# ipastore/glue-factory-colon

Measured on AMD Instinct MI355X. Metric: image-pairs/sec (SuperPoint+LightGlue, 1024 kpts, 640x480), higher is better.
Workload: dtype f32; 1 GPU; SuperPoint-open + LightGlue, 1024 kpts, 640x480 synthetic pairs (BASELINE.json configs[1]); keypoints=1024, parallelism=dp1 (pairs sharded, one final gather), weights=name-seeded seed 0 (no network), pairs_gathered=32, rccl_ranks=1

## Files before the change

glue-factory-colon_amd/csrc/conv_wino43.hip:

```cpp
#include "common.h"

#define S4_TW 32
#define S4_TH 16
#define S4_PR 18
#define S4_PC 34
#define S4_PITCH 36
#define S4_KC 16
#define S4_PLANE (S4_PR * S4_PITCH * 8)
#define S4_PATCH (2 * S4_PLANE)
#define S4_NPIX (S4_PR * S4_PC)
#define S4_IMR 20
#define S4_IMC 36
#define S4_EX (6 * 2 * 32 * 32)
#define S4_THREADS 768
#ifndef S4_DIAG
#define S4_DIAG 0
#endif
#if S4_DIAG & 1
static unsigned long long* g_s4_diag = nullptr;
extern "C" void gfc_diag_set_stem43_stamps(void* p) { g_s4_diag = (unsigned long long*)p; }
#define S4_T(v_) const unsigned long long v_ = __builtin_readcyclecounter()
#else
#define S4_T(v_) do {} while (0)
#endif

struct Stem43Args {
  const float* x;
  const float* w;
  const float* bias;
  const float* scale;
  const float* shift;
  float* y;
  int B, H, W;
  int tiles_x, tiles_y;
  const float* w1;
  const float* b1;
  const float* s1;
  const float* t1;
#if S4_DIAG & 1
  unsigned long long* diag;
#endif
};

__global__ void pack_conv3x3_wino43_kernel(const float* __restrict__ w, float* __restrict__ out, int cout, int cin) {
  const int idx = blockIdx.x * blockDim.x + threadIdx.x;
  if (idx >= cout * cin) return;
  const int ci = idx % cin, co = idx / cin;
  double g[3][3];
  for (int r = 0; r < 3; ++r)
    for (int c = 0; c < 3; ++c) g[r][c] = (double)w[((size_t)co * cin + ci) * 9 + r * 3 + c];
  const double G[6][3] = {{1.0 / 4, 0.0, 0.0},           {-1.0 / 6, -1.0 / 6, -1.0 / 6}, {-1.0 / 6, 1.0 / 6, -1.0 / 6},
                          {1.0 / 24, 1.0 / 12, 1.0 / 6}, {1.0 / 24, -1.0 / 12, 1.0 / 6}, {0.0, 0.0, 1.0}};
  double t[6][3];
  for (int i = 0; i < 6; ++i)
    for (int c = 0; c < 3; ++c) t[i][c] = G[i][0] * g[0][c] + G[i][1] * g[1][c] + G[i][2] * g[2][c];
  const int nt = co / 32, l31 = co % 32;
  const int kg = ci / 8, h = (ci % 8) / 4, s = ci % 4;
  const int lane = 32 * h + l31;
  const int nkg = cin / 8, ntn = cout / 32;
  for (int xi = 0; xi < 6; ++xi)
    for (int nu = 0; nu < 6; ++nu) {
      const double u = t[xi][0] * G[nu][0] + t[xi][1] * G[nu][1] + t[xi][2] * G[nu][2];
      const size_t o = ((((((size_t)xi * nkg + kg) * ntn + nt) * 2 + (s >> 1)) * 6 + nu) * 64 + lane) * 2 + (s & 1);
      out[o] = (float)u;
    }
}

extern "C" int gfc_pack_conv3x3_wino43(const float* w_oihw, float* w_packed, int cout, int cin, void* stream) {
  if (!w_oihw || !w_packed || cout != 64 || cin != 64) return GFC_ERR_INVALID;
  const int total = cout * cin;
  hipLaunchKernelGGL(pack_conv3x3_wino43_kernel, dim3((total + 255) / 256), dim3(256), 0, (hipStream_t)stream, w_oihw,
                     w_packed, cout, cin);
  GFC_LAUNCH_CHECK();
  return GFC_OK;
}

__device__ __forceinline__ float4 f4_scale(float s, float4 a) { return make_float4(s * a.x, s * a.y, s * a.z, s * a.w); }
__device__ __forceinline__ float4 f4_fma(float s, float4 a, float4 b) {
  return make_float4(fmaf(s, a.x, b.x), fmaf(s, a.y, b.y), fmaf(s, a.z, b.z), fmaf(s, a.w, b.w));
}
__device__ __forceinline__ float4 f4_addv(float4 a, float4 b) { return make_float4(a.x + b.x, a.y + b.y, a.z + b.z, a.w + b.w); }
__device__ __forceinline__ float4 f4_subv(float4 a, float4 b) { return make_float4(a.x - b.x, a.y - b.y, a.z - b.z, a.w - b.w); }
__device__ __forceinline__ float4 f4_max(float4 a, float4 b) {
  return make_float4(fmaxf(a.x, b.x), fmaxf(a.y, b.y), fmaxf(a.z, b.z), fmaxf(a.w, b.w));
}

typedef float v2f __attribute__((ext_vector_type(2)));
__device__ __forceinline__ v2f v2_fma(float s, v2f a, v2f b) { return v2f{fmaf(s, a.x, b.x), fmaf(s, a.y, b.y)}; }
__device__ __forceinline__ v2f v2_mul(float s, v2f a) { return v2f{s * a.x, s * a.y}; }
typedef const volatile __attribute__((address_space(3))) v2f* lds_v2f_ptr;
__device__ __forceinline__ v2f lds_pair(const float* p) { return *(lds_v2f_ptr)(p); }

__global__ __launch_bounds__(S4_THREADS, 1) void stem_wino43_kernel(Stem43Args args) {
  const float* const a_x = args.x;
  const float* const a_w = args.w;
  float* const a_y = args.y;
  const int a_B = args.B, a_H = args.H, a_W = args.W, a_tiles_x = args.tiles_x, a_tiles_y = args.tiles_y;
  extern __shared__ __attribute__((aligned(16))) float smem[];
  float* bufA = smem;
  float* bufB = smem + S4_PATCH;
  float* bufC = smem + 2 * S4_PATCH;
  float* img_s = smem + 2 * S4_PATCH + S4_EX;
  float* c1_s = img_s + S4_IMR * S4_IMC;
  float* c2_s = c1_s + 768;

  const int tid = threadIdx.x, lane = tid & 63;
  const int wave = __builtin_amdgcn_readfirstlane(tid >> 6);
  const int xi = wave % 6, nt = wave / 6;
  const int phase = wave >> 2;
  const int l31 = lane & 31, h = lane >> 5;
  const int ty = l31 >> 3, tx = l31 & 7;

  const int per_img = a_tiles_x * a_tiles_y;
  const int nitems = per_img * a_B;

  for (int i = tid; i < 768; i += S4_THREADS)
    c1_s[i] = i < 576 ? args.w1[i] : i < 640 ? args.b1[i - 576] : i < 704 ? (args.s1 ? args.s1[i - 640] : 1.f)
                                                                       : (args.t1 ? args.t1[i - 704] : 0.f);

  if (tid < 192)
    c2_s[tid] = tid < 64 ? args.bias[tid] : tid < 128 ? (args.scale ? args.scale[tid - 64] : 1.f) : (args.shift ? args.shift[tid - 128] : 0.f);

  auto load_img = [&](int it) __attribute__((always_inline)) -> float {
    int t_ = tid;
    asm volatile("" : "+v"(t_));
    const int im_r = (t_ * 1821) >> 16, im_c = t_ - im_r * S4_IMC;
    if (t_ >= S4_IMR * S4_IMC || it >= nitems) return 0.f;
    const int b = it / per_img, t = it - b * per_img;
    const int gy = (t / a_tiles_x) * S4_TH - 2 + im_r, gx = (t % a_tiles_x) * S4_TW - 2 + im_c;
    return (gy >= 0 && gy < a_H && gx >= 0 && gx < a_W) ? a_x[((size_t)b * a_H + gy) * a_W + gx] : 0.f;
  };

  const float2* wbase = reinterpret_cast<const float2*>(a_w) + (size_t)(xi * 32 + nt * 2) * 6 * 64;
  auto bfrag = [&](int hk, int nu) __attribute__((always_inline)) -> float2 {
    const float2* blk = wbase + (size_t)((hk >> 1) * 4 + (hk & 1)) * 6 * 64;
    return blk[nu * 64 + lane];
  };

  const bool three = xi == 0 || xi == 5;
  const int rP = three ? (xi == 0 ? 0 : 1) : (xi == 3 ? 3 : 1);
  const int rQ = three ? rP + 2 : (xi == 1 || xi == 2 ? 2 : (xi == 3 ? 1 : 3));
  const int rR = three ? rP + 4 : (xi == 1 ? 3 : 4);
  const int rS = xi == 1 ? 4 : (xi == 2 ? 3 : 2);
  const float c0 = three ? 4.f : (xi == 1 ? -4.f : xi == 2 ? 4.f : 2.f);
  const float c1 = three ? -5.f : (xi == 1 ? 1.f : -1.f);
  const float c2 = xi == 1 ? 1.f : -1.f;
  const int pix0 = (4 * ty * S4_PITCH + tx) * 8;
  const int offA = pix0 + 2 * ((2 * h) ^ ty), offB = pix0 + 2 * ((2 * h) ^ ((ty + 1) & 3));
  constexpr int COLOFF[6] = {0, 9 * 8, 18 * 8, 27 * 8, 1 * 8, 10 * 8};
  const int ro0 = rP * S4_PITCH * 8, ro1 = rQ * S4_PITCH * 8, ro2 = rR * S4_PITCH * 8, ro3 = rS * S4_PITCH * 8;
  const bool hiR = rR >= 4, hiS = rS >= 4;

#if S4_DIAG & 1
  unsigned long long dg[10] = {0, 0, 0, 0, 0, 0, 0, 0, 0, 0};
  const unsigned long long dg_t0 = __builtin_readcyclecounter();
#endif
  auto conv1a_unit = [&](int u, int ntile, int y0, int x0, float* dst_lo, float* dst_hi) __attribute__((always_inline)) {
    int ln = lane;
    asm volatile("" : "+v"(ln));
    S4_T(tc0);
    const int l31 = ln & 31, h = ln >> 5;
    const int ch = 32 * ntile + l31;
    const float* cb = c1_s + h * 64 + ch;
    const bool edge = u >= 18;
    const int idx_in = min(32 * (u - 18) + l31, 35);
    const float* ip = img_s + (edge ? (idx_in >> 1) * S4_IMC + 32 + (idx_in & 1) : u * S4_IMC + l31);
    f32x16 d;
#pragma unroll
    for (int r = 0; r < 16; ++r) d[r] = 0.f;
    constexpr int T0[5] = {0, 2, S4_IMC + 1, 2 * S4_IMC, 2 * S4_IMC + 2};
    constexpr int T1[5] = {1, S4_IMC, S4_IMC + 2, 2 * S4_IMC + 1, 2 * S4_IMC + 2};
#pragma unroll
    for (int s = 0; s < 5; ++s) {
      const float a0 = ip[T0[s]], a1 = s == 4 ? 1.f : ip[T1[s]];
      d = mfma32(h ? a1 : a0, cb[s * 128], d);
    }
    const float sc = c1_s[640 + ch], sh = c1_s[704 + ch];
#if S4_DIAG & 1
    float probe_ = fmaxf(d[0], 0.f);
    asm volatile("" : "+v"(probe_));
    S4_T(tc1);
    dg[8] += tc1 - tc0;
#endif
    float* dst = (l31 & 16) ? dst_hi : dst_lo;
    const int c16 = l31 & 15;
    const int cofs = (c16 >> 3) * S4_PLANE + (c16 & 1), cpr = (c16 >> 1) & 3;
    if (!edge) {
      const int gy = y0 - 1 + u;
      const bool row_in = gy >= 0 && gy < a_H;
      float* o = dst + cofs + (u * S4_PITCH + h) * 8 + 2 * (cpr ^ ((u >> 2) & 3));
      if (row_in && x0 >= 1 && x0 + 32 < a_W) {
#pragma unroll
        for (int r = 0; r < 16; ++r) {
          const int rr = (r & 3) + 8 * (r >> 2);
          o[((rr & 3) * 9 + (rr >> 2)) * 8] = fmaxf(d[r], 0.f) * sc + sh;
        }
      } else {
        const int gx0 = x0 - 1 + 4 * h;
#pragma unroll
        for (int r = 0; r < 16; ++r) {
          const int rr = (r & 3) + 8 * (r >> 2);
          const float v = (row_in && (unsigned)(gx0 + rr) < (unsigned)a_W) ? fmaxf(d[r], 0.f) * sc + sh : 0.f;
          o[((rr & 3) * 9 + (rr >> 2)) * 8] = v;
        }
      }
    } else {
      const int ib = 32 * (u - 18) + 4 * h;
#pragma unroll
      for (int r = 0; r < 16; ++r) {
        const int idx = ib + (r & 3) + 8 * (r >> 2);
        const bool real = idx < 36;
        const int p = real ? idx >> 1 : 17, cpos = real ? 8 + 9 * (idx & 1) : 35;
        const int gy = y0 - 1 + p, gx = x0 + 31 + (idx & 1);
        const float v = (gy >= 0 && gy < a_H && gx < a_W) ? fmaxf(d[r], 0.f) * sc + sh : 0.f;
        dst[cofs + (p * S4_PITCH + cpos) * 8 + 2 * (cpr ^ ((p >> 2) & 3))] = v;
      }
    }
  };
  auto conv1a_at_half = [&](int half, int ntile, int y0, int x0, float* dst_lo, float* dst_hi) __attribute__((always_inline)) {
    if (half == phase) conv1a_unit(wave, ntile, y0, x0, dst_lo, dst_hi);
    else if (half == phase + 1 && wave + 12 < 20) conv1a_unit(wave + 12, ntile, y0, x0, dst_lo, dst_hi);
  };
  int item = blockIdx.x;
  int y0, x0, b;
  {
    const float v0 = load_img(item);
    if (tid < S4_IMR * S4_IMC) img_s[tid] = v0;
    b = item / per_img;
    const int t_ = item - b * per_img;
    y0 = (t_ / a_tiles_x) * S4_TH; x0 = (t_ % a_tiles_x) * S4_TW;
    __syncthreads();
#pragma unroll 1
    for (int half = 0; half < 4; ++half) conv1a_at_half(half, 0, y0, x0, bufA, bufB);
  }
  float imv = load_img(item + gridDim.x);
  __syncthreads();

  for (; item < nitems; item += gridDim.x) {
    S4_T(t_top);
#if S4_DIAG & 1
    unsigned long long t_prev = t_top;
#endif
    const int nitem = item + gridDim.x;
    const bool have_next = nitem < nitems;
    const int nb_ = nitem / per_img, nt_ = nitem - nb_ * per_img;
    const int ny0 = (nt_ / a_tiles_x) * S4_TH, nx0 = (nt_ % a_tiles_x) * S4_TW;

    f32x16 acc[6];
#pragma unroll
    for (int nu = 0; nu < 6; ++nu)
#pragma unroll
      for (int r = 0; r < 16; ++r) acc[nu][r] = 0.f;

#pragma unroll 1
    for (int c = 0; c < 4; ++c) {
      const float* ps = (c & 1) == 0 ? (c == 0 ? bufA : bufA) : (c == 1 ? bufB : bufC);
      if (c == 2) {
        if (tid < S4_IMR * S4_IMC) img_s[tid] = imv;
        imv = load_img(nitem + gridDim.x);
      }
      S4_T(te);
#if S4_DIAG & 1
      unsigned long long cv_cycles = 0;
      dg[0] += te - t_prev;
#endif
#pragma unroll 1
      for (int half = 0; half < 4; ++half) {
        const int g = half >> 1, hh = half & 1;
        if ((c & 1) && (c == 1 || have_next)) {
          S4_T(tu);
          conv1a_at_half(half, c == 1 ? 1 : 0, c == 1 ? y0 : ny0, c == 1 ? x0 : nx0, bufA, c == 1 ? bufC : bufB);
#if S4_DIAG & 1
          cv_cycles += __builtin_readcyclecounter() - tu;
#endif
        }
        __builtin_amdgcn_sched_barrier(0);
        S4_T(tha);
        float2 bq[6];
#pragma unroll
        for (int nu = 0; nu < 6; ++nu) bq[nu] = bfrag(4 * c + half, nu);
        const float* pl = ps + g * S4_PLANE;
        const float* pA = pl + (offA ^ (2 * hh));
        const float* pB = pl + (offB ^ (2 * hh));
        const float* q0 = pA + ro0;
        const float* q1 = pA + ro1;
        const float* q2 = (hiR ? pB : pA) + ro2;
        const float* q3 = (hiS ? pB : pA) + ro3;
        v2f tr[6];
        if (three) {
          v2f d[2][3];
#pragma unroll
          for (int j = 0; j < 2; ++j) { d[j][0] = lds_pair(q0 + COLOFF[j]); d[j][1] = lds_pair(q1 + COLOFF[j]); d[j][2] = lds_pair(q2 + COLOFF[j]); }
#pragma unroll
          for (int j = 0; j < 6; ++j) {
            __builtin_amdgcn_sched_barrier(0);
            tr[j] = v2_fma(c1, d[j & 1][1], v2_mul(c0, d[j & 1][0])) + d[j & 1][2];
            if (j + 2 < 6) { d[j & 1][0] = lds_pair(q0 + COLOFF[j + 2]); d[j & 1][1] = lds_pair(q1 + COLOFF[j + 2]); d[j & 1][2] = lds_pair(q2 + COLOFF[j + 2]); }
          }
        } else {
          v2f d[2][4];
#pragma unroll
          for (int j = 0; j < 2; ++j) {
            d[j][0] = lds_pair(q0 + COLOFF[j]); d[j][1] = lds_pair(q1 + COLOFF[j]);
            d[j][2] = lds_pair(q2 + COLOFF[j]); d[j][3] = lds_pair(q3 + COLOFF[j]);
          }
#pragma unroll
          for (int j = 0; j < 6; ++j) {
            __builtin_amdgcn_sched_barrier(0);
            tr[j] = v2_fma(c0, v2_fma(c1, d[j & 1][1], d[j & 1][0]), v2_fma(c2, d[j & 1][3], d[j & 1][2]));
            if (j + 2 < 6) {
              d[j & 1][0] = lds_pair(q0 + COLOFF[j + 2]); d[j & 1][1] = lds_pair(q1 + COLOFF[j + 2]);
              d[j & 1][2] = lds_pair(q2 + COLOFF[j + 2]); d[j & 1][3] = lds_pair(q3 + COLOFF[j + 2]);
            }
          }
        }
        __builtin_amdgcn_sched_barrier(0);
        v2f v[6];
        {
          const v2f s12 = tr[1] + tr[2], d12 = tr[1] - tr[2], s34 = tr[3] + tr[4], d34 = tr[3] - tr[4];
          const v2f e31 = tr[3] - tr[1], e42 = tr[4] - tr[2];
          v[0] = v2_fma(-5.f, tr[2], v2_fma(4.f, tr[0], tr[4]));
          v[1] = v2_fma(-4.f, s12, s34);
          v[2] = v2_fma(4.f, d12, -d34);
          v[3] = v2_fma(2.f, e31, e42);
          v[4] = v2_fma(-2.f, e31, e42);
          v[5] = v2_fma(-5.f, tr[3], v2_fma(4.f, tr[1], tr[5]));
        }
#if S4_DIAG & 1
        asm volatile("" : "+v"(v[0]), "+v"(v[5]));
        S4_T(thb);
#endif
#pragma unroll
        for (int nu = 0; nu < 6; nu += 2) {
          acc[nu] = mfma32(v[nu].x, bq[nu].x, acc[nu]);
          acc[nu + 1] = mfma32(v[nu + 1].x, bq[nu + 1].x, acc[nu + 1]);
          acc[nu] = mfma32(v[nu].y, bq[nu].y, acc[nu]);
          acc[nu + 1] = mfma32(v[nu + 1].y, bq[nu + 1].y, acc[nu + 1]);
        }
#if S4_DIAG & 1
        {
          S4_T(thc);
          dg[1] += thb - tha; dg[2] += thc - thb;
        }
#endif
      }
      S4_T(tg);
      __syncthreads();
      S4_T(th);
#if S4_DIAG & 1
      dg[3] += cv_cycles; dg[4] += tg - te - cv_cycles; dg[5] += th - tg;
      t_prev = th;
#endif
    }
    S4_T(ti);

    float* ex = bufC;
    int tq = tid;
    asm volatile("" : "+v"(tq));
    const int co_q = (tq & 7) * 4, ip2 = (tq >> 3) & 1, tile = tq >> 4;
    const int Ho = a_H >> 1, Wo = a_W >> 1;
#pragma unroll 1
    for (int pnt = 0; pnt < 2; ++pnt)
#pragma unroll
    for (int jp = 0; jp < 2; ++jp) {
      if (nt == pnt) {
        int ln = lane;
        asm volatile("" : "+v"(ln));
        float* ob = ex + xi * 2048 + 4 * (ln >> 5) * 32 + (ln & 31);
#pragma unroll
        for (int r = 0; r < 16; ++r) {
          const float m1 = acc[1][r], m2 = acc[2][r], m3 = acc[3][r], m4 = acc[4][r];
          const float s12 = m1 + m2, d12 = m1 - m2, s34 = m3 + m4, d34 = m3 - m4;
          float* o = ob + ((r & 3) + 8 * (r >> 2)) * 32;
          if (jp == 0) {
            o[0] = (acc[0][r] + s12) + s34;
            o[1024] = fmaf(2.f, d34, d12);
          } else {
            o[0] = fmaf(4.f, s34, s12);
            o[1024] = fmaf(8.f, d34, d12) + acc[5][r];
          }
        }
      }
      __syncthreads();
      if (tid < 512) {
        const int co = pnt * 32 + co_q;
        const float kd = ip2 ? 8.f : 2.f;
        float4 pool = make_float4(0.f, 0.f, 0.f, 0.f);
#pragma unroll
        for (int jj = 0; jj < 2; ++jj) {
          __builtin_amdgcn_sched_barrier(0);
          const float* zp = ex + jj * 1024 + tile * 32 + co_q;
          const float4 z1 = *reinterpret_cast<const float4*>(zp + 2048);
          const float4 z2 = *reinterpret_cast<const float4*>(zp + 2 * 2048);
          const float4 s12 = f4_addv(z1, z2), d12 = f4_subv(z1, z2);
          __builtin_amdgcn_sched_barrier(0);
          const float4 z3 = *reinterpret_cast<const float4*>(zp + 3 * 2048);
          const float4 z4 = *reinterpret_cast<const float4*>(zp + 4 * 2048);
          const float4 s34 = f4_addv(z3, z4), d34 = f4_subv(z3, z4);
          __builtin_amdgcn_sched_barrier(0);
          const float4 ze = *reinterpret_cast<const float4*>(zp + (ip2 ? 5 * 2048 : 0));
          float4 ya = ip2 ? f4_fma(4.f, s34, s12) : f4_addv(f4_addv(ze, s12), s34);
          float4 yb = f4_fma(kd, d34, d12);
          if (ip2) yb = f4_addv(yb, ze);
          const float4 bi = *reinterpret_cast<const float4*>(c2_s + co);
          const float4 sc = *reinterpret_cast<const float4*>(c2_s + 64 + co);
          const float4 sh = *reinterpret_cast<const float4*>(c2_s + 128 + co);
          float4 t = f4_addv(ya, bi);
          t = make_float4(fmaxf(t.x, 0.f), fmaxf(t.y, 0.f), fmaxf(t.z, 0.f), fmaxf(t.w, 0.f));
          ya = make_float4(t.x * sc.x + sh.x, t.y * sc.y + sh.y, t.z * sc.z + sh.z, t.w * sc.w + sh.w);
          t = f4_addv(yb, bi);
          t = make_float4(fmaxf(t.x, 0.f), fmaxf(t.y, 0.f), fmaxf(t.z, 0.f), fmaxf(t.w, 0.f));
          yb = make_float4(t.x * sc.x + sh.x, t.y * sc.y + sh.y, t.z * sc.z + sh.z, t.w * sc.w + sh.w);
          const float4 m = f4_max(ya, yb);
          pool = jj == 0 ? m : f4_max(pool, m);
        }
        const int oy = (y0 >> 1) + 2 * (tile >> 3) + ip2, ox = (x0 >> 1) + 2 * (tile & 7) + jp;
        if (ox < Wo && oy < Ho) *reinterpret_cast<float4*>(a_y + (((size_t)b * Ho + oy) * Wo + ox) * 64 + co) = pool;
      }
      __syncthreads();
    }
#if S4_DIAG & 1
    {
      S4_T(tj);
      dg[6] += tj - ti; dg[7] += 1;
    }
#endif
    y0 = ny0; x0 = nx0; b = nb_;
  }
#if S4_DIAG & 1
  if (args.diag && lane == 0) {
    unsigned long long* o = args.diag + ((size_t)blockIdx.x * 12 + wave) * 16;
    for (int i = 0; i < 8; ++i) o[i] = dg[i];
    o[8] = __builtin_readcyclecounter() - dg_t0;
    o[9] = dg[8];
  }
#endif
}

extern "C" int gfc_sp_stem_wino43(const float* image, const float* w1, const float* b1, const float* s1, const float* t1,
                                  const float* w2_wino43, const float* b2, const float* s2, const float* t2, float* y,
                                  int B, int H, int W, void* stream) {
  if (!image || !w1 || !b1 || !w2_wino43 || !b2 || !y || B <= 0 || H < 2 || W < 2) return GFC_ERR_INVALID;
  if ((s1 == nullptr) != (t1 == nullptr) || (s2 == nullptr) != (t2 == nullptr)) return GFC_ERR_INVALID;
  Stem43Args a = {};
  a.x = image; a.w = w2_wino43; a.bias = b2; a.scale = s2; a.shift = t2; a.y = y;
  a.B = B; a.H = H; a.W = W;
  a.w1 = w1; a.b1 = b1; a.s1 = s1; a.t1 = t1;
  a.tiles_x = (W + S4_TW - 1) / S4_TW;
  a.tiles_y = (H + S4_TH - 1) / S4_TH;
  const long long nitems = (long long)a.tiles_x * a.tiles_y * B;
  if (nitems >= (1ll << 31)) return GFC_ERR_UNSUPPORTED;
  constexpr size_t lds = (size_t)(2 * S4_PATCH + S4_EX + S4_IMR * S4_IMC + 768 + 192) * sizeof(float);
  static_assert(S4_EX >= S4_PATCH, "patch buffer C is the head of the exchange buffer");
  static std::atomic<unsigned long long> lds_ok{0};
  gfc_allow_dynamic_lds((const void*)stem_wino43_kernel, lds, lds_ok);
  long long grid = gfc_device_cus();
  if (grid > nitems) grid = nitems;
#if S4_DIAG & 1
  a.diag = g_s4_diag;
#endif
  hipLaunchKernelGGL(stem_wino43_kernel, dim3((unsigned)grid), dim3(S4_THREADS), lds, (hipStream_t)stream, a);
  GFC_LAUNCH_CHECK();
  return GFC_OK;
}
```

Measured before the change: 930.9 image-pairs/sec.

## Switch Winograd stem GEMM from 32x32x1 to 16x16x4 MFMA with new LDS layout

Replaces the 32x32x1 f32 MFMA accumulation in the fused SuperPoint stem Winograd F(4,3) kernel with 16x16x4 f32 MFMA. The packed weight layout, LDS patch layout (per-channel planes with padded strides instead of interleaved 8-channel pixels with XOR swizzle) and the output exchange/pooling indexing are all reworked to match the new fragment shapes. Each wave now owns an M-half of tiles across all 64 output channels rather than half the channels. The intent is higher MFMA throughput and fewer bank conflicts, at the cost of scalar rather than paired LDS loads and more accumulator registers.

Result: no change. 937.5 image-pairs/sec (median of 6 runs) (+0.7%).

```diff
diff --git a/glue-factory-colon_amd/csrc/conv_wino43.hip b/glue-factory-colon_amd/csrc/conv_wino43.hip
--- a/glue-factory-colon_amd/csrc/conv_wino43.hip
+++ b/glue-factory-colon_amd/csrc/conv_wino43.hip
@@ -6,8 +6,13 @@
 #define S4_PC 34
 #define S4_PITCH 36
 #define S4_KC 16
-#define S4_PLANE (S4_PR * S4_PITCH * 8)
-#define S4_PATCH (2 * S4_PLANE)
+#define S4_CH1 (S4_PR * S4_PITCH)
+#define S4_CH2 (2 * S4_CH1 + 17)
+#define S4_CHOFS(c) ((((c) >> 2) & 1) * S4_CH1 + (((c) & 3) + 4 * ((c) >> 3)) * S4_CH2)
+#define S4_KQOFS(kq) (((kq) & 1) * S4_CH1 + ((kq) >> 1) * S4_CH2)
+#define S4_PATCH (8 * S4_CH2)
+#define S4_BUFB 10512
+#define S4_BUFC 21040
 #define S4_NPIX (S4_PR * S4_PC)
 #define S4_IMR 20
 #define S4_IMC 36
@@ -54,14 +59,14 @@
   double t[6][3];
   for (int i = 0; i < 6; ++i)
     for (int c = 0; c < 3; ++c) t[i][c] = G[i][0] * g[0][c] + G[i][1] * g[1][c] + G[i][2] * g[2][c];
-  const int nt = co / 32, l31 = co % 32;
-  const int kg = ci / 8, h = (ci % 8) / 4, s = ci % 4;
-  const int lane = 32 * h + l31;
-  const int nkg = cin / 8, ntn = cout / 32;
+  const int n = co / 16, r8 = ci % 8;
+  const int k4 = 2 * (ci / 8) + ((r8 & 3) >> 1), kq = 2 * (r8 & 1) + (r8 >> 2);
+  const int lane = 16 * kq + co % 16;
+  const int nk4 = cin / 4;
   for (int xi = 0; xi < 6; ++xi)
     for (int nu = 0; nu < 6; ++nu) {
       const double u = t[xi][0] * G[nu][0] + t[xi][1] * G[nu][1] + t[xi][2] * G[nu][2];
-      const size_t o = ((((((size_t)xi * nkg + kg) * ntn + nt) * 2 + (s >> 1)) * 6 + nu) * 64 + lane) * 2 + (s & 1);
+      const size_t o = ((((size_t)xi * nk4 + k4) * 6 + nu) * 64 + lane) * 4 + n;
       out[o] = (float)u;
     }
 }
@@ -85,11 +90,9 @@
   return make_float4(fmaxf(a.x, b.x), fmaxf(a.y, b.y), fmaxf(a.z, b.z), fmaxf(a.w, b.w));
 }
 
-typedef float v2f __attribute__((ext_vector_type(2)));
-__device__ __forceinline__ v2f v2_fma(float s, v2f a, v2f b) { return v2f{fmaf(s, a.x, b.x), fmaf(s, a.y, b.y)}; }
-__device__ __forceinline__ v2f v2_mul(float s, v2f a) { return v2f{s * a.x, s * a.y}; }
-typedef const volatile __attribute__((address_space(3))) v2f* lds_v2f_ptr;
-__device__ __forceinline__ v2f lds_pair(const float* p) { return *(lds_v2f_ptr)(p); }
+__device__ __forceinline__ f32x4 mfma16(float a, float b, f32x4 c) {
+  return __builtin_amdgcn_mfma_f32_16x16x4f32(a, b, c, 0, 0, 0);
+}
 
 __global__ __launch_bounds__(S4_THREADS, 1) void stem_wino43_kernel(Stem43Args args) {
   const float* const a_x = args.x;
@@ -98,18 +101,18 @@
   const int a_B = args.B, a_H = args.H, a_W = args.W, a_tiles_x = args.tiles_x, a_tiles_y = args.tiles_y;
   extern __shared__ __attribute__((aligned(16))) float smem[];
   float* bufA = smem;
-  float* bufB = smem + S4_PATCH;
-  float* bufC = smem + 2 * S4_PATCH;
-  float* img_s = smem + 2 * S4_PATCH + S4_EX;
+  float* bufB = smem + S4_BUFB;
+  float* bufC = smem + S4_BUFC;
+  float* img_s = smem + S4_BUFC + S4_EX;
   float* c1_s = img_s + S4_IMR * S4_IMC;
   float* c2_s = c1_s + 768;
 
   const int tid = threadIdx.x, lane = tid & 63;
   const int wave = __builtin_amdgcn_readfirstlane(tid >> 6);
-  const int xi = wave % 6, nt = wave / 6;
+  const int xi = wave % 6, mh = wave / 6;
   const int phase = wave >> 2;
-  const int l31 = lane & 31, h = lane >> 5;
-  const int ty = l31 >> 3, tx = l31 & 7;
+  const int l15 = lane & 15, kq = lane >> 4;
+  const int ty = 2 * mh + (l15 >> 3), tx = l15 & 7;
 
   const int per_img = a_tiles_x * a_tiles_y;
   const int nitems = per_img * a_B;
@@ -131,10 +134,10 @@
     return (gy >= 0 && gy < a_H && gx >= 0 && gx < a_W) ? a_x[((size_t)b * a_H + gy) * a_W + gx] : 0.f;
   };
 
-  const float2* wbase = reinterpret_cast<const float2*>(a_w) + (size_t)(xi * 32 + nt * 2) * 6 * 64;
-  auto bfrag = [&](int hk, int nu) __attribute__((always_inline)) -> float2 {
-    const float2* blk = wbase + (size_t)((hk >> 1) * 4 + (hk & 1)) * 6 * 64;
-    return blk[nu * 64 + lane];
+  const float4* wbase = reinterpret_cast<const float4*>(a_w) + (size_t)xi * 16 * 6 * 64;
+  auto bfrag = [&](int k4, int nu, int ln) __attribute__((always_inline)) -> float4 {
+    const float4* blk = wbase + (size_t)k4 * 6 * 64;
+    return blk[nu * 64 + ln];
   };
 
   const bool three = xi == 0 || xi == 5;
@@ -142,22 +145,22 @@
   const int rQ = three ? rP + 2 : (xi == 1 || xi == 2 ? 2 : (xi == 3 ? 1 : 3));
   const int rR = three ? rP + 4 : (xi == 1 ? 3 : 4);
   const int rS = xi == 1 ? 4 : (xi == 2 ? 3 : 2);
-  const float c0 = three ? 4.f : (xi == 1 ? -4.f : xi == 2 ? 4.f : 2.f);
-  const float c1 = three ? -5.f : (xi == 1 ? 1.f : -1.f);
-  const float c2 = xi == 1 ? 1.f : -1.f;
-  const int pix0 = (4 * ty * S4_PITCH + tx) * 8;
-  const int offA = pix0 + 2 * ((2 * h) ^ ty), offB = pix0 + 2 * ((2 * h) ^ ((ty + 1) & 3));
-  constexpr int COLOFF[6] = {0, 9 * 8, 18 * 8, 27 * 8, 1 * 8, 10 * 8};
-  const int ro0 = rP * S4_PITCH * 8, ro1 = rQ * S4_PITCH * 8, ro2 = rR * S4_PITCH * 8, ro3 = rS * S4_PITCH * 8;
-  const bool hiR = rR >= 4, hiS = rS >= 4;
+  auto uniform = [](float x) __attribute__((always_inline)) { return __int_as_float(__builtin_amdgcn_readfirstlane(__float_as_int(x))); };
+  const float c0 = uniform(three ? 4.f : (xi == 1 ? -4.f : xi == 2 ? 4.f : 2.f));
+  const float c1 = uniform(three ? -5.f : (xi == 1 ? 1.f : -1.f));
+  const float c2 = uniform(xi == 1 ? 1.f : -1.f);
+  const int off0 = S4_KQOFS(kq) + 4 * ty * S4_PITCH + tx;
+  constexpr int COLOFF[6] = {0, 9, 18, 27, 1, 10};
+  const int ro0 = rP * S4_PITCH, ro1 = rQ * S4_PITCH, ro2 = rR * S4_PITCH, ro3 = rS * S4_PITCH;
 
 #if S4_DIAG & 1
   unsigned long long dg[10] = {0, 0, 0, 0, 0, 0, 0, 0, 0, 0};
   const unsigned long long dg_t0 = __builtin_readcyclecounter();
 #endif
   auto conv1a_unit = [&](int u, int ntile, int y0, int x0, float* dst_lo, float* dst_hi) __attribute__((always_inline)) {
-    int ln = lane;
+    int ln = tid;
     asm volatile("" : "+v"(ln));
+    ln &= 63;
     S4_T(tc0);
     const int l31 = ln & 31, h = ln >> 5;
     const int ch = 32 * ntile + l31;
@@ -184,16 +187,16 @@
 #endif
     float* dst = (l31 & 16) ? dst_hi : dst_lo;
     const int c16 = l31 & 15;
-    const int cofs = (c16 >> 3) * S4_PLANE + (c16 & 1), cpr = (c16 >> 1) & 3;
+    const int cofs = S4_CHOFS(c16);
     if (!edge) {
       const int gy = y0 - 1 + u;
       const bool row_in = gy >= 0 && gy < a_H;
-      float* o = dst + cofs + (u * S4_PITCH + h) * 8 + 2 * (cpr ^ ((u >> 2) & 3));
+      float* o = dst + cofs + u * S4_PITCH + h;
       if (row_in && x0 >= 1 && x0 + 32 < a_W) {
 #pragma unroll
         for (int r = 0; r < 16; ++r) {
           const int rr = (r & 3) + 8 * (r >> 2);
-          o[((rr & 3) * 9 + (rr >> 2)) * 8] = fmaxf(d[r], 0.f) * sc + sh;
+          o[(rr & 3) * 9 + (rr >> 2)] = fmaxf(d[r], 0.f) * sc + sh;
         }
       } else {
         const int gx0 = x0 - 1 + 4 * h;
@@ -201,7 +204,7 @@
         for (int r = 0; r < 16; ++r) {
           const int rr = (r & 3) + 8 * (r >> 2);
           const float v = (row_in && (unsigned)(gx0 + rr) < (unsigned)a_W) ? fmaxf(d[r], 0.f) * sc + sh : 0.f;
-          o[((rr & 3) * 9 + (rr >> 2)) * 8] = v;
+          o[(rr & 3) * 9 + (rr >> 2)] = v;
         }
       }
     } else {
@@ -213,7 +216,7 @@
         const int p = real ? idx >> 1 : 17, cpos = real ? 8 + 9 * (idx & 1) : 35;
         const int gy = y0 - 1 + p, gx = x0 + 31 + (idx & 1);
         const float v = (gy >= 0 && gy < a_H && gx < a_W) ? fmaxf(d[r], 0.f) * sc + sh : 0.f;
-        dst[cofs + (p * S4_PITCH + cpos) * 8 + 2 * (cpr ^ ((p >> 2) & 3))] = v;
+        dst[cofs + p * S4_PITCH + cpos] = v;
       }
     }
   };
@@ -246,17 +249,19 @@
     const int nb_ = nitem / per_img, nt_ = nitem - nb_ * per_img;
     const int ny0 = (nt_ / a_tiles_x) * S4_TH, nx0 = (nt_ % a_tiles_x) * S4_TW;
 
-    f32x16 acc[6];
+    f32x4 acc[6][4];
 #pragma unroll
     for (int nu = 0; nu < 6; ++nu)
 #pragma unroll
-      for (int r = 0; r < 16; ++r) acc[nu][r] = 0.f;
+      for (int n = 0; n < 4; ++n) acc[nu][n] = f32x4{0.f, 0.f, 0.f, 0.f};
 
 #pragma unroll 1
     for (int c = 0; c < 4; ++c) {
       const float* ps = (c & 1) == 0 ? (c == 0 ? bufA : bufA) : (c == 1 ? bufB : bufC);
       if (c == 2) {
-        if (tid < S4_IMR * S4_IMC) img_s[tid] = imv;
+        int tw = tid;
+        asm volatile("" : "+v"(tw));
+        if (tw < S4_IMR * S4_IMC) img_s[tw] = imv;
         imv = load_img(nitem + gridDim.x);
       }
       S4_T(te);
@@ -266,7 +271,6 @@
 #endif
 #pragma unroll 1
       for (int half = 0; half < 4; ++half) {
-        const int g = half >> 1, hh = half & 1;
         if ((c & 1) && (c == 1 || have_next)) {
           S4_T(tu);
           conv1a_at_half(half, c == 1 ? 1 : 0, c == 1 ? y0 : ny0, c == 1 ? x0 : nx0, bufA, c == 1 ? bufC : bufB);
@@ -276,66 +280,69 @@
         }
         __builtin_amdgcn_sched_barrier(0);
         S4_T(tha);
-        float2 bq[6];
-#pragma unroll
-        for (int nu = 0; nu < 6; ++nu) bq[nu] = bfrag(4 * c + half, nu);
-        const float* pl = ps + g * S4_PLANE;
-        const float* pA = pl + (offA ^ (2 * hh));
-        const float* pB = pl + (offB ^ (2 * hh));
-        const float* q0 = pA + ro0;
-        const float* q1 = pA + ro1;
-        const float* q2 = (hiR ? pB : pA) + ro2;
-        const float* q3 = (hiS ? pB : pA) + ro3;
-        v2f tr[6];
+        float4 bq[6];
+        int lnw = tid;
+        asm volatile("" : "+v"(lnw));
+        lnw &= 63;
+#pragma unroll
+        for (int nu = 0; nu < 6; ++nu) bq[nu] = bfrag(4 * c + half, nu, lnw);
+        int o0 = off0;
+        asm volatile("" : "+v"(o0));
+        const float* pl = ps + half * (2 * S4_CH2) + o0;
+        const float* q0 = pl + ro0;
+        const float* q1 = pl + ro1;
+        const float* q2 = pl + ro2;
+        const float* q3 = pl + ro3;
+        float tr[6];
         if (three) {
-          v2f d[2][3];
-#pragma unroll
-          for (int j = 0; j < 2; ++j) { d[j][0] = lds_pair(q0 + COLOFF[j]); d[j][1] = lds_pair(q1 + COLOFF[j]); d[j][2] = lds_pair(q2 + COLOFF[j]); }
+          float d[2][3];
+#pragma unroll
+          for (int j = 0; j < 2; ++j) { d[j][0] = q0[COLOFF[j]]; d[j][1] = q1[COLOFF[j]]; d[j][2] = q2[COLOFF[j]]; }
 #pragma unroll
           for (int j = 0; j < 6; ++j) {
             __builtin_amdgcn_sched_barrier(0);
-            tr[j] = v2_fma(c1, d[j & 1][1], v2_mul(c0, d[j & 1][0])) + d[j & 1][2];
-            if (j + 2 < 6) { d[j & 1][0] = lds_pair(q0 + COLOFF[j + 2]); d[j & 1][1] = lds_pair(q1 + COLOFF[j + 2]); d[j & 1][2] = lds_pair(q2 + COLOFF[j + 2]); }
+            tr[j] = fmaf(c1, d[j & 1][1], c0 * d[j & 1][0]) + d[j & 1][2];
+            if (j + 2 < 6) { d[j & 1][0] = q0[COLOFF[j + 2]]; d[j & 1][1] = q1[COLOFF[j + 2]]; d[j & 1][2] = q2[COLOFF[j + 2]]; }
           }
         } else {
-          v2f d[2][4];
+          float d[2][4];
 #pragma unroll
           for (int j = 0; j < 2; ++j) {
-            d[j][0] = lds_pair(q0 + COLOFF[j]); d[j][1] = lds_pair(q1 + COLOFF[j]);
-            d[j][2] = lds_pair(q2 + COLOFF[j]); d[j][3] = lds_pair(q3 + COLOFF[j]);
+            d[j][0] = q0[COLOFF[j]]; d[j][1] = q1[COLOFF[j]];
+            d[j][2] = q2[COLOFF[j]]; d[j][3] = q3[COLOFF[j]];
           }
 #pragma unroll
           for (int j = 0; j < 6; ++j) {
             __builtin_amdgcn_sched_barrier(0);
-            tr[j] = v2_fma(c0, v2_fma(c1, d[j & 1][1], d[j & 1][0]), v2_fma(c2, d[j & 1][3], d[j & 1][2]));
+            tr[j] = fmaf(c0, fmaf(c1, d[j & 1][1], d[j & 1][0]), fmaf(c2, d[j & 1][3], d[j & 1][2]));
             if (j + 2 < 6) {
-              d[j & 1][0] = lds_pair(q0 + COLOFF[j + 2]); d[j & 1][1] = lds_pair(q1 + COLOFF[j + 2]);
-              d[j & 1][2] = lds_pair(q2 + COLOFF[j + 2]); d[j & 1][3] = lds_pair(q3 + COLOFF[j + 2]);
+              d[j & 1][0] = q0[COLOFF[j + 2]]; d[j & 1][1] = q1[COLOFF[j + 2]];
+              d[j & 1][2] = q2[COLOFF[j + 2]]; d[j & 1][3] = q3[COLOFF[j + 2]];
             }
           }
         }
         __builtin_amdgcn_sched_barrier(0);
-        v2f v[6];
+        float v[6];
         {
-          const v2f s12 = tr[1] + tr[2], d12 = tr[1] - tr[2], s34 = tr[3] + tr[4], d34 = tr[3] - tr[4];
-          const v2f e31 = tr[3] - tr[1], e42 = tr[4] - tr[2];
-          v[0] = v2_fma(-5.f, tr[2], v2_fma(4.f, tr[0], tr[4]));
-          v[1] = v2_fma(-4.f, s12, s34);
-          v[2] = v2_fma(4.f, d12, -d34);
-          v[3] = v2_fma(2.f, e31, e42);
-          v[4] = v2_fma(-2.f, e31, e42);
-          v[5] = v2_fma(-5.f, tr[3], v2_fma(4.f, tr[1], tr[5]));
+          const float s12 = tr[1] + tr[2], d12 = tr[1] - tr[2], s34 = tr[3] + tr[4], d34 = tr[3] - tr[4];
+          const float e31 = tr[3] - tr[1], e42 = tr[4] - tr[2];
+          v[0] = fmaf(-5.f, tr[2], fmaf(4.f, tr[0], tr[4]));
+          v[1] = fmaf(-4.f, s12, s34);
+          v[2] = fmaf(4.f, d12, -d34);
+          v[3] = fmaf(2.f, e31, e42);
+          v[4] = fmaf(-2.f, e31, e42);
+          v[5] = fmaf(-5.f, tr[3], fmaf(4.f, tr[1], tr[5]));
         }
 #if S4_DIAG & 1
         asm volatile("" : "+v"(v[0]), "+v"(v[5]));
         S4_T(thb);
 #endif
 #pragma unroll
-        for (int nu = 0; nu < 6; nu += 2) {
-          acc[nu] = mfma32(v[nu].x, bq[nu].x, acc[nu]);
-          acc[nu + 1] = mfma32(v[nu + 1].x, bq[nu + 1].x, acc[nu + 1]);
-          acc[nu] = mfma32(v[nu].y, bq[nu].y, acc[nu]);
-          acc[nu + 1] = mfma32(v[nu + 1].y, bq[nu + 1].y, acc[nu + 1]);
+        for (int nu = 0; nu < 6; ++nu) {
+          acc[nu][0] = mfma16(v[nu], bq[nu].x, acc[nu][0]);
+          acc[nu][1] = mfma16(v[nu], bq[nu].y, acc[nu][1]);
+          acc[nu][2] = mfma16(v[nu], bq[nu].z, acc[nu][2]);
+          acc[nu][3] = mfma16(v[nu], bq[nu].w, acc[nu][3]);
         }
 #if S4_DIAG & 1
         {
@@ -355,41 +362,49 @@
     S4_T(ti);
 
     float* ex = bufC;
-    int tq = tid;
-    asm volatile("" : "+v"(tq));
-    const int co_q = (tq & 7) * 4, ip2 = (tq >> 3) & 1, tile = tq >> 4;
     const int Ho = a_H >> 1, Wo = a_W >> 1;
-#pragma unroll 1
+#pragma unroll
     for (int pnt = 0; pnt < 2; ++pnt)
 #pragma unroll
     for (int jp = 0; jp < 2; ++jp) {
-      if (nt == pnt) {
-        int ln = lane;
+      {
+        int ln = tid;
         asm volatile("" : "+v"(ln));
-        float* ob = ex + xi * 2048 + 4 * (ln >> 5) * 32 + (ln & 31);
-#pragma unroll
-        for (int r = 0; r < 16; ++r) {
-          const float m1 = acc[1][r], m2 = acc[2][r], m3 = acc[3][r], m4 = acc[4][r];
-          const float s12 = m1 + m2, d12 = m1 - m2, s34 = m3 + m4, d34 = m3 - m4;
-          float* o = ob + ((r & 3) + 8 * (r >> 2)) * 32;
-          if (jp == 0) {
-            o[0] = (acc[0][r] + s12) + s34;
-            o[1024] = fmaf(2.f, d34, d12);
-          } else {
-            o[0] = fmaf(4.f, s34, s12);
-            o[1024] = fmaf(8.f, d34, d12) + acc[5][r];
+        ln &= 63;
+        float* ob = ex + xi * 2048 + (16 * mh + 4 * (ln >> 4)) * 32 + (ln & 15);
+        const int swz = (ln >> 4) & 1;
+#pragma unroll
+        for (int nn = 0; nn < 2; ++nn) {
+          float* on = ob + 16 * (nn ^ swz);
+#pragma unroll
+          for (int r = 0; r < 4; ++r) {
+            const int n = 2 * pnt + nn;
+            const float m1 = acc[1][n][r], m2 = acc[2][n][r], m3 = acc[3][n][r], m4 = acc[4][n][r];
+            const float s12 = m1 + m2, d12 = m1 - m2, s34 = m3 + m4, d34 = m3 - m4;
+            float* o = on + r * 32;
+            if (jp == 0) {
+              o[0] = (acc[0][n][r] + s12) + s34;
+              o[1024] = fmaf(2.f, d34, d12);
+            } else {
+              o[0] = fmaf(4.f, s34, s12);
+              o[1024] = fmaf(8.f, d34, d12) + acc[5][n][r];
+            }
           }
         }
       }
       __syncthreads();
-      if (tid < 512) {
+      int tq = tid;
+      asm volatile("" : "+v"(tq));
+      const int co_q = (tq & 7) * 4, ip2 = (tq >> 3) & 1, tile = tq >> 4;
+      const int oy = (y0 >> 1) + 2 * (tile >> 3) + ip2, ox = (x0 >> 1) + 2 * (tile & 7) + jp;
+      if (tq < 512 && ox < Wo && oy < Ho) {
         const int co = pnt * 32 + co_q;
         const float kd = ip2 ? 8.f : 2.f;
         float4 pool = make_float4(0.f, 0.f, 0.f, 0.f);
 #pragma unroll
         for (int jj = 0; jj < 2; ++jj) {
           __builtin_amdgcn_sched_barrier(0);
-          const float* zp = ex + jj * 1024 + tile * 32 + co_q;
+          const float* zp = ex + jj * 1024 + tile * 32 + (co_q ^ ((tile & 4) << 2));
           const float4 z1 = *reinterpret_cast<const float4*>(zp + 2048);
           const float4 z2 = *reinterpret_cast<const float4*>(zp + 2 * 2048);
           const float4 s12 = f4_addv(z1, z2), d12 = f4_subv(z1, z2);
@@ -414,8 +429,10 @@
           const float4 m = f4_max(ya, yb);
           pool = jj == 0 ? m : f4_max(pool, m);
         }
-        const int oy = (y0 >> 1) + 2 * (tile >> 3) + ip2, ox = (x0 >> 1) + 2 * (tile & 7) + jp;
-        if (ox < Wo && oy < Ho) *reinterpret_cast<float4*>(a_y + (((size_t)b * Ho + oy) * Wo + ox) * 64 + co) = pool;
+        int ts = tid;
+        asm volatile("" : "+v"(ts));
+        const int oy_s = (y0 >> 1) + 2 * (ts >> 7) + ((ts >> 3) & 1), ox_s = (x0 >> 1) + 2 * ((ts >> 4) & 7) + jp;
+        *reinterpret_cast<float4*>(a_y + (((size_t)b * Ho + oy_s) * Wo + ox_s) * 64 + pnt * 32 + (ts & 7) * 4) = pool;
       }
       __syncthreads();
     }
@@ -450,8 +467,10 @@
   a.tiles_y = (H + S4_TH - 1) / S4_TH;
   const long long nitems = (long long)a.tiles_x * a.tiles_y * B;
   if (nitems >= (1ll << 31)) return GFC_ERR_UNSUPPORTED;
-  constexpr size_t lds = (size_t)(2 * S4_PATCH + S4_EX + S4_IMR * S4_IMC + 768 + 192) * sizeof(float);
+  constexpr size_t lds = (size_t)(S4_BUFC + S4_EX + S4_IMR * S4_IMC + 768 + 192) * sizeof(float);
   static_assert(S4_EX >= S4_PATCH, "patch buffer C is the head of the exchange buffer");
+  static_assert(S4_BUFB >= S4_PATCH && S4_BUFC - S4_BUFB >= S4_PATCH && S4_BUFB % 32 == 16 && S4_BUFC % 32 == 16,
+                "patch buffers are disjoint and half a bank row apart");
   static std::atomic<unsigned long long> lds_ok{0};
   gfc_allow_dynamic_lds((const void*)stem_wino43_kernel, lds, lds_ok);
   long long grid = gfc_device_cus();
```
